# thegenemyers/DEXTRACTOR

Measured on AMD Instinct MI355X. Metric: dexqv encode input GB/s (5 QV/tag stream bytes per base; .dexqv bit-exact vs reference), higher is better.
Workload: dtype u8

## Files before the change

dextractor_amd/csrc/dx_qv.hip:

```cpp
#include "dx_internal.hpp"
#include "dx_device.hpp"

#ifndef HIST_NT
#define HIST_NT 0
#endif
#if HIST_NT
#define HIST_LOAD(p) __builtin_nontemporal_load((const u32x4_u *) (p))
#else
#define HIST_LOAD(p) (*(const u32x4_u *) (p))
#endif

#define TOK_LEN(e)  ((e) >> 26)
#define TOK_BITS(e) ((e) & 0xffffffu)
#define TOK_ESC(e)  (((e) >> 25) & 1u)
#define TOK_PACK(bits, len, esc) (((bits) & 0xffffffu) | ((uint32_t) (len) << 26) | ((esc) ? 0x2000000u : 0u))

#define QV_WIN_WORDS  512
#define QV_WIN_BITS   (32u * (QV_WIN_WORDS - 32))
#define QV_WIN_PAD    4
#ifndef QV_FLUSH_BITS
#define QV_FLUSH_BITS 8192u
#endif
#define TAG_WIN_WORDS 128
#define TAG_FLUSH_BITS 1024u

#ifndef SIZES_WAVES
#define SIZES_WAVES 4
#endif
#ifndef ENC_WAVES
#define ENC_WAVES 4
#endif
#ifndef HIST_SKIP
#define HIST_SKIP 0
#endif
#ifndef HIST_TRIM
#define HIST_TRIM 0
#endif

struct qv_args
{ const uint8_t  *text;
  const uint64_t *off;
  const uint32_t *len;
  uint64_t        n;
  uint64_t        text_bytes;
  uint32_t        pad;
  int             delChar, subChar;
  int             lossy;
  uint32_t        units;
};

static uint32_t ticket_units(uint64_t bytes, uint64_t n, uint32_t target, uint32_t least)
{ if (n == 0 || bytes == 0) return least;
  const uint64_t mean = bytes / n + 1u;
  uint64_t u = ((uint64_t) target + mean - 1u) / mean;
  return (uint32_t) (u < least ? least : (u > 4096u ? 4096u : u));
}

__device__ __forceinline__ const uint8_t *line_ptr(const qv_args &a, uint64_t r, uint32_t L, int k)
{ return a.text + a.off[r] + (uint64_t) k * ((uint64_t) L + a.pad); }

__device__ __forceinline__ bool can_overread(const qv_args &a, const uint8_t *p, uint32_t L)
{ return (uint64_t) (p - a.text) + L + 16u <= a.text_bytes; }

__device__ __forceinline__ u32x4 fetch(const uint8_t *p, uint32_t pos, uint32_t L, bool over)
{ u32x4 v = { 0u, 0u, 0u, 0u };
  if (pos < L)
    { const uint32_t left = L - pos;
      if (left >= 16u)
        v = *(const u32x4_u *) (p + pos);
      else if (over)
        { v = *(const u32x4_u *) (p + pos);
          const uint32_t m0 = left >= 4u  ? ~0u : ~(~0u << (8u * left));
          const uint32_t m1 = left >= 8u  ? ~0u : (left > 4u  ? ~(~0u << (8u * (left - 4u)))  : 0u);
          const uint32_t m2 = left >= 12u ? ~0u : (left > 8u  ? ~(~0u << (8u * (left - 8u)))  : 0u);
          const uint32_t m3 =                     (left > 12u ? ~(~0u << (8u * (left - 12u))) : 0u);
          v.x &= m0; v.y &= m1; v.z &= m2; v.w &= m3;
        }
      else
        v = load_chunk(p + pos, (int) left);
    }
  return v;
}

__device__ __forceinline__ int valid_of(uint32_t pos, uint32_t L)
{ return pos >= L ? 0 : (L - pos >= 16u ? 16 : (int) (L - pos)); }

__device__ __forceinline__ u32x4 fetch_step(const uint8_t *p, uint32_t base, uint32_t L, bool over)
{ const uint32_t pos = base + 16u * (uint32_t) lane_id();
  if (base + DX_STEP <= L)
    return *(const u32x4_u *) (p + pos);
  return fetch(p, pos, L, over);
}

#define BYTE_OF(c, b) ((chunk_word(c, (b) >> 2) >> (8 * ((b) & 3))) & 0xffu)

struct run_lds
{ uint8_t  *chunk;
  uint16_t *list;
};

__device__ __forceinline__ uint32_t run_collect(const run_lds &R, const u32x4 &c, int valid, uint32_t rc)
{ const int lane = lane_id();
  uint32_t       nr   = ~chunk_eq_mask(c, rc) & ((1u << valid) - 1u);
  const uint32_t cnt  = __popc(nr);
  const uint32_t incl = wave_incl_scan(cnt);
  uint32_t       idx  = incl - cnt;
  *(u32x4 *) (R.chunk + 16 * lane) = c;
  const uint32_t p16 = 16u * (uint32_t) lane;
  if (HIST_SKIP & 4) nr = 0;
  while (nr)
    { R.list[idx++] = (uint16_t) (p16 + (uint32_t) __builtin_ctz(nr));
      nr &= nr - 1u;
    }
  wave_sync();
  return wave_total(incl);
}

__device__ __forceinline__ uint32_t run_after(const run_lds &R, uint32_t total, uint32_t sv, uint32_t C)
{ return total ? sv - 1u - (uint32_t) R.list[total - 1] : C + sv; }


__global__ __launch_bounds__(DX_BLOCK)
void k_qv_prescan_del(qv_args a, uint64_t entry0, unsigned long long *key)
{ const int      lane  = lane_id();
  const uint64_t wave0 = (uint64_t) blockIdx.x * DX_WAVES_PER_BLK + (threadIdx.x >> 6);
  const uint64_t nwave = (uint64_t) gridDim.x * DX_WAVES_PER_BLK;

  for (uint64_t r = wave0; r < a.n; r += nwave)
    { const unsigned long long cur = __hip_atomic_load(key, __ATOMIC_RELAXED, __HIP_MEMORY_SCOPE_AGENT);
      if (entry0 + r >= (cur >> 8))
        break;
      const uint32_t L   = a.len[r];
      const uint8_t *del = line_ptr(a, r, L, 0);
      const uint8_t *tag = line_ptr(a, r, L, 1);
      bool found = false, done = false;
      for (uint32_t base = 0; base < L && !done; base += DX_STEP)
        { const uint32_t pos   = base + 16u * lane;
          const int      valid = valid_of(pos, L);
          const u32x4    c     = load_chunk(tag + pos, valid);
          const uint32_t m     = (chunk_eq_mask(c, 'n') | chunk_eq_mask(c, 'N')) & ((1u << valid) - 1u);
          const uint64_t any   = __ballot(m != 0);
          if (any)
            { const int      f = __ffsll((unsigned long long) any) - 1;
              const uint32_t k = pos + (uint32_t) (m ? __ffs(m) - 1 : 0);
              const uint32_t d = __shfl((uint32_t) (lane == f ? del[k] : 0u), f);
              done  = true;
              found = d < 128u;
              if (found && lane == f)
                atomicMin(key, ((unsigned long long) (entry0 + r) << 8) | d);
            }
        }
      if (found)
        break;
    }
}

__global__ __launch_bounds__(DX_BLOCK)
void k_qv_prescan_sub(qv_args a, long long *out )
{ __shared__ uint32_t s_hist[256];
  __shared__ uint64_t s_part[DX_BLOCK];
  __shared__ long long s_first;
  const int tid = threadIdx.x;

  s_hist[tid] = 0;
  if (tid == 0) s_first = -1;
  __syncthreads();

  uint64_t running = 0;
  for (uint64_t c0 = 0; c0 < a.n; c0 += DX_BLOCK)
    { const uint64_t i = c0 + tid;
      s_part[tid] = i < a.n ? a.len[i] : 0;
      __syncthreads();
      if (tid == 0)
        for (int k = 0; k < DX_BLOCK && c0 + k < a.n; k++)
          { running += s_part[k];
            if (running >= 100000ull)
              { s_first = (long long) (c0 + k);
                break;
              }
          }
      __syncthreads();
      if (s_first >= 0)
        break;
    }
  const long long first = s_first;
  if (first < 0)
    { if (tid == 0) { out[0] = -1; out[1] = -1; }
      return;
    }

  const int lane = lane_id(), wid = tid >> 6;
  for (long long r = wid; r <= first; r += DX_WAVES_PER_BLK)
    { const uint32_t L    = a.len[r];
      const uint8_t *sub  = line_ptr(a, (uint64_t) r, L, 4);
      const bool     over = can_overread(a, sub, L);
      for (uint32_t base = 0; base < L; base += DX_STEP)
        { const uint32_t pos   = base + 16u * (uint32_t) lane;
          const u32x4    c     = fetch(sub, pos, L, over);
          const int      valid = valid_of(pos, L);
          for (int b = 0; b < valid; b++)
            atomicAdd(&s_hist[chunk_byte(c, b)], 1u);
        }
    }
  __syncthreads();
  if (tid == 0)
    { int best = 0;
      for (int k = 1; k < 256; k++)
        if (s_hist[k] > s_hist[best])
          best = k;
      out[0] = first;
      out[1] = best;
    }
}

#ifndef TICKET_BATCH
#define TICKET_BATCH 2u
#endif
#ifndef HIST_BLOCK
#define HIST_BLOCK   1024
#endif
#ifndef HIST_PER_CU
#define HIST_PER_CU  1
#endif
#define HIST_NWAVE   (HIST_BLOCK / 64)
#ifndef HC_PLAIN
#define HC_PLAIN     32
#endif
#ifndef HC_RSYM
#define HC_RSYM      8
#endif
#ifndef HC_RUN
#define HC_RUN       8
#endif
#define HSYM_FAST    128
#define HRUN_FAST    128
#ifndef HIST_BARE_FETCH
#define HIST_BARE_FETCH 1
#endif

struct hist_lds
{ uint32_t plain[2][HSYM_FAST][HC_PLAIN];
  uint32_t rsym[2][HSYM_FAST][HC_RSYM];
  uint32_t run[2][HRUN_FAST][HC_RUN];
  uint32_t slow[6][256];
};
#define HIST_W_PLAIN (2 * HSYM_FAST * HC_PLAIN)
#define HIST_W_RSYM  (2 * HSYM_FAST * HC_RSYM)
#define HIST_W_RUN   (2 * HRUN_FAST * HC_RUN)
#define HIST_FAST_WORDS (HIST_W_PLAIN + HIST_W_RSYM + HIST_W_RUN)

template <int COLS>
__device__ __forceinline__ void hist_plain_step(const u32x4 &c, int valid, bool full, uint32_t (*h)[COLS], uint32_t *slow)
{ const uint32_t col = (uint32_t) lane_id() & (COLS - 1);
  const bool wide = __any((int) ((c.x | c.y | c.z | c.w) & 0x80808080u));
  if (full && !wide)
    {
      #pragma unroll
      for (int b = 0; b < 16; b++)
        atomicAdd(&h[BYTE_OF(c, b)][col], 1u);
    }
  else
    for (int b = 0; b < valid; b++)
      { const uint32_t x = chunk_byte(c, b);
        if (x < HSYM_FAST) atomicAdd(&h[x][col], 1u);
        else               atomicAdd(&slow[x], 1u);
      }
}

#define TOK_RUN_MAX  127u
#define TOK_BAD      0x80000000u
#define TOK_INFO     8u
#define TOK_XMARGIN  40u

struct tok_sink
{ uint16_t       *del, *sub;
  const uint64_t *off;
  uint32_t       *info;
  unsigned long long *unusable;
  uint32_t       *list;
};

__host__ __device__ __forceinline__ uint32_t tok_room(uint32_t L, uint32_t fr8)
{ return (((uint32_t) (((uint64_t) L * fr8) >> 8) + 64u + TOK_XMARGIN) + 7u) & ~7u; }

__device__ __forceinline__ uint32_t tok_exception_at(const uint32_t *slot_end, uint32_t nx, uint32_t idx)
{ uint32_t lo = 0, hi = nx;
  while (lo < hi)
    { const uint32_t mid = (lo + hi) >> 1;
      if (*(slot_end - 2 * (int) mid - 2) < idx) lo = mid + 1; else hi = mid;
    }
  return lo;
}
__device__ __forceinline__ uint32_t tok_exception(const uint32_t *slot_end, uint32_t nx, uint32_t idx)
{ return *(slot_end - 2 * (int) tok_exception_at(slot_end, nx, idx) - 1); }

__device__ __forceinline__ bool tok_unusable(const uint32_t *info, uint64_t r, int delChar, int subChar)
{ return (delChar >= 0 && (info[TOK_INFO * r] & TOK_BAD)) || (subChar >= 0 && (info[TOK_INFO * r + 1] & TOK_BAD)); }

__device__ __forceinline__ uint32_t chunk_ne_mask(const u32x4 &v, uint32_t c4 )
{ uint32_t p[4];
  #pragma unroll
  for (int i = 0; i < 4; i++)
    { const uint32_t w = chunk_word(v, i) ^ c4;
      p[i] = ((((w & 0x7f7f7f7fu) + 0x7f7f7f7fu) | w) & 0x80808080u) * 0x00204081u;
    }
  const uint32_t even = __builtin_amdgcn_perm(p[2], p[0], 0x0c0c0703u);
  const uint32_t odd  = __builtin_amdgcn_perm(p[3], p[1], 0x0c0c0703u);
  return (even >> 4) | odd;
}

__device__ __forceinline__ uint32_t chunk_byte_sel(const u32x4 &v, uint32_t selA, uint32_t selB)
{ return __builtin_amdgcn_perm(__builtin_amdgcn_perm(v.w, v.z, selA), __builtin_amdgcn_perm(v.y, v.x, selA), selB); }

__device__ __forceinline__ uint32_t wave_shr1(uint32_t v)
{ return (uint32_t) __builtin_amdgcn_update_dpp(0u, v, 0x138, 0xf, 0xf, true); }

struct tok_pend { uint64_t v; uint32_t n, at; };

__device__ __forceinline__ void tok_flush(tok_pend &p, uint16_t *tok)
{ if (4u * (uint32_t) lane_id() < p.n)
    *(u64_u *) (tok + p.at + 4u * (uint32_t) lane_id()) = p.v;
  p.n = 0;
}

__device__ __forceinline__ uint32_t tag_code(uint32_t letter)
{ const uint32_t i = min((letter & 0xdfu) - 0x41u, 31u);
  return (uint32_t) (((1ull << 4) | (2ull << 12) | (3ull << 38)) >> (2u * i)) & 3u;
}

struct hist_wave_lds
{ uint8_t  chunk[DX_STEP], tags[DX_STEP];
  uint16_t list[DX_STEP];
};
#ifndef PPC_INS
#define PPC_INS 8
#endif
#ifndef PPC_MRG
#define PPC_MRG 4
#endif
#ifndef HIST_LIST
#define HIST_LIST 512
#endif
struct hist_wave_own
{ uint32_t pi[128][PPC_INS], pm[128][PPC_MRG];
#ifndef PSC
#define PSC 1
#endif
  uint32_t ps[2][128][PSC];
#ifndef PRC
#define PRC 1
#endif
  uint32_t pr[2][128][PRC];
  uint16_t list[HIST_LIST];
};
#define EH_WORDS 384u

template <bool TAGS, bool OWN, bool LDSX>
__device__ __forceinline__ void hist_runs_step(hist_wave_lds *W, uint16_t *wlist, const u32x4 &c, const u32x4 &t, uint32_t vmask, uint32_t sv, uint32_t rc4,
                                               uint32_t &C, uint32_t &nrun, uint32_t *hs, uint32_t *slow_s,
                                               uint32_t *hr, uint32_t *slow_r, uint32_t inc,
                                               uint16_t *tok, uint32_t &ntok, uint32_t room, uint32_t &bad, uint32_t &nexc,
                                               tok_pend &pend_out)
{ constexpr uint32_t HCS = OWN ? (uint32_t) PSC : HC_RSYM, HCR = OWN ? (uint32_t) PRC : HC_RUN;
  const uint32_t lane  = (uint32_t) lane_id();
  const uint32_t nr0   = chunk_ne_mask(c, rc4) & vmask;
  const uint32_t cnt   = __popc(nr0);
  const uint32_t incl  = wave_incl_scan(cnt);
  const uint32_t total = wave_total(incl);
  nrun += sv - total;
  if (LDSX)
    { *(u32x4 *) (W->chunk + 16u * lane) = c;
      if (TAGS) *(u32x4 *) (W->tags + 16u * lane) = t;
    }
  const bool fits = OWN ? total <= (uint32_t) HIST_LIST : true;
  const bool emit = !(HIST_SKIP & 8) && !bad && fits && ntok + total + 4u * nexc <= room;
  if (!emit) bad = 1;
  const uint32_t tend  = cnt ? 16u * lane + 32u - (uint32_t) __clz(nr0) + C : 0u;
  const uint32_t imax  = wave_incl_max(tend);
  const uint32_t gmax  = __builtin_amdgcn_readlane(imax, 63);
  const uint32_t s0    = wave_shr1(imax) - (16u * lane + C);
  const uint32_t li0   = incl - cnt;
  uint32_t nr = (HIST_SKIP & 1) ? 0u : nr0, s = s0, acc = 0;
  uint16_t      *lp = wlist + (fits ? li0 : 0u);
  const uint8_t *cp = LDSX ? W->chunk + 16u * lane : (const uint8_t *) NULL;
  const uint32_t pinc = OWN ? 1u : inc;
  while (nr)
    { const uint32_t b   = (uint32_t) __builtin_ctz(nr);
      nr &= nr - 1u;
      uint32_t x, tg = 0;
      if (!LDSX)
        { const uint32_t selA = (b & 7u) | 0x0c0c0c00u, selB = ((b >> 1) & 4u) | 0x0c0c0c00u;
          x = chunk_byte_sel(c, selA, selB);
          if (TAGS) tg = chunk_byte_sel(t, selA, selB);
        }
      else
        { x = cp[b];
          if (TAGS) tg = cp[b + DX_STEP];
        }
      const uint32_t run = b - s;
      const uint32_t r7  = run < TOK_RUN_MAX ? run : TOK_RUN_MAX;
      s   = b + 1u;
      acc = max(acc, max(run, x));
#if HIST_TRIM
      const uint32_t x4 = x << 2;
      atomicAdd((uint32_t *) ((uint8_t *) hs + (x4 & (4u * (HSYM_FAST - 1))) * HCS), 1u);
      atomicAdd(&hr[r7 * HCR], pinc);
      uint32_t tk = (r7 << 9) | x4;
      if (TAGS) tk |= tag_code(tg);
#else
      atomicAdd(&hs[(x & (HSYM_FAST - 1)) * HCS], 1u);
      atomicAdd(&hr[r7 * HCR], pinc);
      uint32_t tk = x | (r7 << 7);
      if (TAGS) tk = (tk << 2) | tag_code(tg);
      else      tk <<= 2;
#endif
      *lp++ = (uint16_t) tk;
    }
  uint32_t odd = 0;
  if (__any((int) (acc >= TOK_RUN_MAX)))
    { uint32_t m = nr0, ne = 0;
      s = s0;
      while (m)
        { const uint32_t b   = (uint32_t) __builtin_ctz(m);
          m &= m - 1u;
          const uint32_t x   = LDSX ? (uint32_t) cp[b] : chunk_byte(c, (int) b);
          const uint32_t run = b - s;
          s = b + 1u;
          if (run >= TOK_RUN_MAX)
            { atomicSub(&hr[TOK_RUN_MAX * HCR], pinc);
              atomicAdd(&slow_r[run > 255u ? 255u : run], inc);
              ne++;
            }
          if (x >= HSYM_FAST)
            { atomicSub(&hs[(x & (HSYM_FAST - 1)) * HCS], 1u);
              atomicAdd(&slow_s[x], 1u);
              odd = 1;
            }
        }
      if (emit && __any((int) ne))
        { const uint32_t ince = wave_incl_scan(ne);
          uint32_t  j    = nexc + ince - ne, i = ntok + li0;
          uint32_t *xend = (uint32_t *) (tok + room + TOK_XMARGIN);
          m = nr0; s = s0;
          while (m)
            { const uint32_t b   = (uint32_t) __builtin_ctz(m);
              m &= m - 1u;
              const uint32_t run = b - s;
              s = b + 1u;
              if (run >= TOK_RUN_MAX)
                { *(xend - 2 * (int) j - 2) = i;
                  *(xend - 2 * (int) j - 1) = run;
                  j++;
                }
              i++;
            }
          nexc += wave_total(ince);
        }
      else if (OWN && __any((int) ne))
        bad = 1;
    }
  if (emit)
    { __builtin_amdgcn_wave_barrier();
      if (HIST_SKIP & 32) { }
      else if (total <= 256u)
        { pend_out.v = *(const uint64_t *) (wlist + 4u * lane); pend_out.n = total; pend_out.at = ntok; }
      else
        for (uint32_t i = 4u * lane; i < total; i += 256u)
          *(u64_u *) (tok + ntok + i) = *(const uint64_t *) (wlist + i);
      ntok += total;
      if (__any((int) odd)) bad = 1;
    }
  C = sv + C - gmax;
  __builtin_amdgcn_wave_barrier();
}

__device__ __forceinline__ void hist_plain_pair(const u32x4 &c2, const u32x4 &c3, int valid, bool full, hist_lds &H)
{ const uint32_t col = (uint32_t) lane_id() & (HC_PLAIN - 1);
  if (full && !__any((int) ((c2.x | c2.y | c2.z | c2.w | c3.x | c3.y | c3.z | c3.w) & 0x80808080u)))
    {
      #pragma unroll
      for (int b = 0; b < 16; b++)
        atomicAdd(&H.plain[0][BYTE_OF(c2, b)][col], 1u);
      #pragma unroll
      for (int b = 0; b < 16; b++)
        atomicAdd(&H.plain[1][BYTE_OF(c3, b)][col], 1u);
    }
  else
    { hist_plain_step<HC_PLAIN>(c2, valid, full, H.plain[0], H.slow[DX_INS]);
      hist_plain_step<HC_PLAIN>(c3, valid, full, H.plain[1], H.slow[DX_MRG]);
    }
}

__device__ __forceinline__ uint32_t hist_plain_pair_own(const u32x4 &c2, const u32x4 &c3, int valid, bool full, uint32_t *pi, uint32_t *pm,
                                                        uint32_t *slow_ins, uint32_t *slow_mrg)
{ uint32_t *const q0 = pi + ((uint32_t) lane_id() & (PPC_INS - 1u)), *const q1 = pm + ((uint32_t) lane_id() & (PPC_MRG - 1u));
#define OWN_ADD(q, x) atomicAdd(&(q)[((q) == q0 ? (uint32_t) PPC_INS : (uint32_t) PPC_MRG) * (x)], 1u)
  if (!__any((int) ((c2.x | c2.y | c2.z | c2.w | c3.x | c3.y | c3.z | c3.w) & 0x80808080u)))
    { if (full || valid > 0)
        {
          #pragma unroll
          for (int b = 0; b < 16; b++)
            OWN_ADD(q0, BYTE_OF(c2, b));
          #pragma unroll
          for (int b = 0; b < 16; b++)
            OWN_ADD(q1, BYTE_OF(c3, b));
          if (!full && valid < 16)
            { atomicSub(&q0[0], (uint32_t) (16 - valid));
              atomicSub(&q1[0], (uint32_t) (16 - valid));
            }
        }
      return 0;
    }
  for (int b = 0; b < valid; b++)
    { const uint32_t x = chunk_byte(c2, b), y = chunk_byte(c3, b);
      if (x < 128u) OWN_ADD(q0, x);
      else          atomicAdd(&slow_ins[x], 1u);
      if (y < 128u) OWN_ADD(q1, y);
      else          atomicAdd(&slow_mrg[y], 1u);
    }
#undef OWN_ADD
  return 1;
}

__device__ __forceinline__ uint32_t hist_bin_of(uint32_t k)
{ if (k < HIST_W_PLAIN)
    return (DX_INS + k / (HSYM_FAST * HC_PLAIN)) * 256u + (k / HC_PLAIN) % HSYM_FAST;
  k -= HIST_W_PLAIN;
  if (k < HIST_W_RSYM)
    return (k / (HSYM_FAST * HC_RSYM) ? DX_SUB : DX_DEL) * 256u + (k / HC_RSYM) % HSYM_FAST;
  k -= HIST_W_RSYM;
  if (k < HIST_W_RUN)
    return (4u + k / (HRUN_FAST * HC_RUN)) * 256u + (k / HC_RUN) % HRUN_FAST;
  return k - HIST_W_RUN;
}

__device__ __forceinline__ uint32_t hist_copies_of(uint32_t k)
{ return k < HIST_W_PLAIN ? HC_PLAIN : (k < HIST_W_PLAIN + HIST_W_RSYM ? HC_RSYM : HC_RUN); }

struct meta_row { const uint8_t *base; uint32_t stride, pad; };

__device__ __forceinline__ uint32_t meta_load(const meta_row *s_meta, uint32_t words, uint64_t r)
{ uint32_t v = 0;
  const uint32_t lane = (uint32_t) lane_id();
  if (lane < words)
    { const meta_row m = s_meta[lane];
      v = *(const uint32_t *) (m.base + r * m.stride);
    }
  return v;
}
#define META(m, k)   ((uint32_t) __builtin_amdgcn_readlane((int) (m), (int) (k)))
#define META64(m, k) ((uint64_t) META(m, k) | ((uint64_t) META(m, (k) + 1) << 32))

struct scan_dev
{ int32_t   delChar, subChar;
  long long del_first, sub_first;
  uint32_t  inst;
  uint32_t  share8;
};
#define SCAN_G     0u
#define SCAN_A     1u
#define SCAN_B     2u
#define SCAN_NOTOK 3u
#define SCAN_MISS  0x100u

template <bool FAST, bool OWNTOK> struct hist_smem;
template <> struct hist_smem<false, false> { hist_lds H; hist_wave_lds W[HIST_NWAVE]; };
template <> struct hist_smem<true, true>   { uint32_t slow[6][256]; hist_wave_own W[HIST_NWAVE]; };
struct hist_wave_plain { uint32_t pi[128][PPC_INS], pm[128][PPC_MRG]; uint16_t list[DX_STEP]; };
template <> struct hist_smem<true, false>
{ uint32_t slow[6][256];
  uint32_t rsym[2][HSYM_FAST][HC_RSYM], run[2][HRUN_FAST][HC_RUN];
  hist_wave_plain W[HIST_NWAVE];
};

template <bool FAST, bool OWNTOK>
__global__ __launch_bounds__(HIST_BLOCK, (HIST_NWAVE * HIST_PER_CU + 3) / 4)
void k_qv_hist(qv_args a, uint64_t entry0, long long del_first, long long sub_first,
               unsigned long long *g_hist , unsigned long long *g_tot, uint32_t *ticket, tok_sink ts, uint32_t *eh ,
               const scan_dev *sd , uint64_t tok_cap ,
               const uint32_t *orig )
{ __shared__ __attribute__((aligned(16))) hist_smem<FAST, OWNTOK> S;
  if (sd != NULL)
    { if (sd->inst != (FAST ? (OWNTOK ? SCAN_A : SCAN_B) : SCAN_G) || ts.off[a.n] > tok_cap)
        return;
      a.delChar = sd->delChar; a.subChar = sd->subChar;
      del_first = sd->del_first; sub_first = sd->sub_first;
    }
  typedef hist_smem<false, false> smem_g;
  typedef hist_smem<true, true>   smem_a;
  typedef hist_smem<true, false>  smem_b;
  const int      lane  = lane_id();
  const int      tid   = threadIdx.x;
  const int      wid   = tid >> 6;
  uint32_t (*const slow)[256] = !FAST ? ((smem_g *) (void *) &S)->H.slow : (OWNTOK ? ((smem_a *) (void *) &S)->slow : ((smem_b *) (void *) &S)->slow);
  hist_lds      *const Hp = FAST ? (hist_lds *) NULL : &((smem_g *) (void *) &S)->H;
  hist_wave_lds *const Wl = FAST ? (hist_wave_lds *) NULL : &((smem_g *) (void *) &S)->W[wid];
  hist_wave_own *const Wo = FAST && OWNTOK ? &((smem_a *) (void *) &S)->W[wid] : (hist_wave_own *) NULL;
  smem_b        *const Sb = FAST && !OWNTOK ? (smem_b *) (void *) &S : (smem_b *) NULL;
  uint32_t *const piw = !FAST ? (uint32_t *) NULL : (OWNTOK ? &Wo->pi[0][0] : &Sb->W[wid].pi[0][0]);
  uint32_t *const pmw = !FAST ? (uint32_t *) NULL : (OWNTOK ? &Wo->pm[0][0] : &Sb->W[wid].pm[0][0]);
  uint16_t      *const wlist = !FAST ? Wl->list : (OWNTOK ? Wo->list : Sb->W[wid].list);
  uint32_t *const words = (uint32_t *) (void *) &S;
  const uint32_t  nwords = sizeof(S) / 4;
  const bool      toks  = FAST || ts.del != NULL;
  constexpr bool OT = FAST && OWNTOK;
  uint32_t (*const rsymp)[HSYM_FAST][HC_RSYM] = FAST ? (OWNTOK ? (uint32_t (*)[HSYM_FAST][HC_RSYM]) NULL : Sb->rsym) : Hp->rsym;
  uint32_t (*const runp)[HRUN_FAST][HC_RUN]   = FAST ? (OWNTOK ? (uint32_t (*)[HRUN_FAST][HC_RUN]) NULL : Sb->run) : Hp->run;
  uint32_t *const hs0 = OT ? &Wo->ps[0][0][(uint32_t) lane & (PSC - 1)] : &rsymp[0][0][(uint32_t) lane & (HC_RSYM - 1)];
  uint32_t *const hs4 = OT ? &Wo->ps[1][0][(uint32_t) lane & (PSC - 1)] : &rsymp[1][0][(uint32_t) lane & (HC_RSYM - 1)];
  uint32_t *const hr0 = OT ? &Wo->pr[0][0][(uint32_t) lane & (PRC - 1)] : &runp[0][0][(uint32_t) lane & (HC_RUN - 1)];
  uint32_t *const hr4 = OT ? &Wo->pr[1][0][(uint32_t) lane & (PRC - 1)] : &runp[1][0][(uint32_t) lane & (HC_RUN - 1)];
  const uint32_t  rc0 = (uint32_t) (a.delChar & 0xff) * 0x01010101u, rc4 = (uint32_t) (a.subChar & 0xff) * 0x01010101u;

#define HM_WORDS 8u
  __shared__ __attribute__((aligned(16))) meta_row s_meta[HM_WORDS];
  if (tid < (int) HM_WORDS)
    { meta_row m;
      if      (tid == 0) { m.base = (const uint8_t *) a.len;                   m.stride = 4u; }
      else if (tid < 3)  { m.base = (const uint8_t *) a.off + 4 * (tid - 1);   m.stride = 8u; }
      else if (tid < 7)  { m.base = (const uint8_t *) ts.off + 4 * (tid - 3);  m.stride = 8u; }
      else               { m.base = (const uint8_t *) orig;                    m.stride = 4u; }
      if ((tid >= 3 && tid < 7 && !(FAST || ts.del != NULL)) || (tid == 7 && orig == NULL))
        { m.base = (const uint8_t *) a.len; m.stride = 0u; }
      m.pad = 0;
      s_meta[tid] = m;
    }
  for (uint32_t k = tid; k < nwords; k += HIST_BLOCK) words[k] = 0;
  __syncthreads();

  uint64_t tot = 0, since = 0;
  uint32_t mpre = 0;
  uint64_t mfor = ~0ull;
  for (uint64_t r0 = next_unit(ticket, a.units), nxt; r0 < a.n; r0 = nxt)
  { nxt = next_unit(ticket, a.units);
    for (uint64_t r = r0; r < r0 + a.units && r < a.n; r++)
    { const uint32_t mw = mfor == r ? mpre : meta_load(s_meta, HM_WORDS, r);
      { const uint64_t rn = r + 1 < r0 + a.units && r + 1 < a.n ? r + 1 : nxt;
        mfor = rn;
        if (rn < a.n) mpre = meta_load(s_meta, HM_WORDS, rn);
      }
      const uint32_t  L = META(mw, 0);
      const long long g = (long long) (entry0 + (orig ? (uint64_t) META(mw, 7) : r));
      const bool drun = FAST || (a.delChar >= 0 && (toks || g >= del_first));
      const bool srun = FAST || (a.subChar >= 0 && (toks || g >= sub_first));
      const uint32_t dinc = (a.delChar >= 0 && g >= del_first) ? 1u : 0u, sinc = (a.subChar >= 0 && g >= sub_first) ? 1u : 0u;
      const uint8_t *p0 = a.text + META64(mw, 1);
      const uint64_t pitch = (uint64_t) L + a.pad;
      const uint8_t *p1 = p0 + pitch, *p2 = p1 + pitch, *p3 = p2 + pitch, *p4 = p3 + pitch;
      const bool over = can_overread(a, p4, L);
      uint32_t C0 = 0, C4 = 0, n0 = 0, n4 = 0;
      uint16_t *tk0 = NULL, *tk4 = NULL;
      uint32_t  nt0 = 0, nt4 = 0, room = 0, bad0 = 0, bad4 = 0, nx0 = 0, nx4 = 0;
      tok_pend  pd0 = { 0ull, 0u, 0u }, pd4 = { 0ull, 0u, 0u };
      if (toks)
        { const uint64_t t0 = META64(mw, 3);
          room = (uint32_t) (META64(mw, 5) - t0) - TOK_XMARGIN;
          if (drun) tk0 = ts.del + t0;
          if (srun) tk4 = ts.sub + t0;
        }
      const bool tags = FAST || tk0 != NULL;

      uint32_t pos = 16u * lane;
      u32x4 c0 = fetch(p0, pos, L, over), c4 = fetch(p4, pos, L, over);
      u32x4 t1 = c0;
      if (tags) t1 = fetch(p1, pos, L, over);
      for (uint32_t base = 0; base < L; base += DX_STEP)
        { const uint32_t np = pos + DX_STEP;
          __builtin_amdgcn_s_waitcnt(0x0F70);
          if (toks)
            { tok_flush(pd0, tk0);
              tok_flush(pd4, tk4);
            }
          u32x4 c2, c3, d0, d4, u1 = c0;
          if (HIST_BARE_FETCH && base + DX_STEP <= L)
            { c2 = HIST_LOAD(p2 + pos); c3 = HIST_LOAD(p3 + pos); }
          else
            { c2 = fetch(p2, pos, L, over); c3 = fetch(p3, pos, L, over); }
          if (HIST_BARE_FETCH && base + 2u * DX_STEP <= L)
            { d0 = HIST_LOAD(p0 + np); d4 = HIST_LOAD(p4 + np);
              if (tags) u1 = HIST_LOAD(p1 + np);
            }
          else
            { d0 = fetch(p0, np, L, over); d4 = fetch(p4, np, L, over);
              if (tags) u1 = fetch(p1, np, L, over);
            }
          const uint32_t sv    = L - base >= DX_STEP ? DX_STEP : L - base;
          const bool     full  = sv == DX_STEP;
          const int      valid = valid_of(pos, L);
          const uint32_t vmask = (1u << valid) - 1u;
          if (HIST_SKIP & 16) { }
          else if (drun) hist_runs_step<true, OT, !FAST>(Wl, wlist, c0, t1, vmask, sv, rc0, C0, n0, hs0, slow[DX_DEL], hr0, slow[DX_DRUN],
                                                    dinc, tk0, nt0, tk0 != NULL ? room : 0u, bad0, nx0, pd0);
          else      hist_plain_step<HC_RSYM>(c0, valid, full, Hp->rsym[0], slow[DX_DEL]);
          if (HIST_SKIP & 16) { }
          else if (srun) hist_runs_step<false, OT, !FAST>(Wl, wlist, c4, c4, vmask, sv, rc4, C4, n4, hs4, slow[DX_SUB], hr4, slow[DX_SRUN],
                                                     sinc, tk4, nt4, tk4 != NULL ? room : 0u, bad4, nx4, pd4);
          else      hist_plain_step<HC_RSYM>(c4, valid, full, Hp->rsym[1], slow[DX_SUB]);
          if (HIST_SKIP & 2) { }
          else if (FAST) bad0 |= hist_plain_pair_own(c2, c3, valid, full, piw, pmw, slow[DX_INS], slow[DX_MRG]);
          else           hist_plain_pair(c2, c3, valid, full, *Hp);
          c0 = d0; c4 = d4; t1 = u1;
          pos = np;
        }
      tok_flush(pd0, tk0);
      tok_flush(pd4, tk4);
      if (FAST)
        {
          __builtin_amdgcn_wave_barrier();
          uint32_t *e32 = eh + (uint64_t) r * EH_WORDS;
          const u32x4 zero = { 0u, 0u, 0u, 0u };
          #pragma unroll
          for (int k = 0; k < 2; k++)
            { const int cp = k == 0 ? PPC_INS : PPC_MRG;
              u32x4 *w = (u32x4 *) ((k == 0 ? piw : pmw) + 2 * lane * cp);
              uint32_t ce = 0, co = 0;
              if (cp == 2)
                { const u32x4 v = w[0];
                  w[0] = zero;
                  ce = v.x + v.y; co = v.z + v.w;
                }
              else
                {
                  #pragma unroll
                  for (int j = 0; j < cp / 4; j++)
                    { const u32x4 v0 = w[j], v1 = w[cp / 4 + j];
                      w[j] = zero; w[cp / 4 + j] = zero;
                      ce += v0.x + v0.y + v0.z + v0.w; co += v1.x + v1.y + v1.z + v1.w;
                    }
                }
              e32[64 * k + lane] = (ce & 0xffffu) | (co << 16);
              if (ce | co)
                { atomicAdd(&slow[DX_INS + k][2 * lane], ce);
                  atomicAdd(&slow[DX_INS + k][2 * lane + 1], co);
                }
            }
          #pragma unroll
          for (int k = 0; k < (OT ? 4 : 0); k++)
            { uint32_t v0, v1;
              if (k < 2)
                { uint32_t *w = &Wo->ps[k][2 * lane][0];
                  v0 = 0; v1 = 0;
                  #pragma unroll
                  for (int j = 0; j < PSC; j++)
                    { v0 += w[j]; v1 += w[PSC + j];
                      w[j] = 0; w[PSC + j] = 0;
                    }
                }
              else
                { uint32_t *w = &Wo->pr[k - 2][2 * lane][0];
                  v0 = 0; v1 = 0;
                  #pragma unroll
                  for (int j = 0; j < PRC; j++)
                    { v0 += w[j]; v1 += w[PRC + j];
                      w[j] = 0; w[PRC + j] = 0;
                    }
                }
              e32[128 + 64 * k + lane] = (v0 & 0xffffu) | (v1 << 16);
              const int      tab = k == 0 ? DX_DEL : (k == 1 ? DX_SUB : (k == 2 ? DX_DRUN : DX_SRUN));
              const uint32_t on  = k == 2 ? dinc : (k == 3 ? sinc : 1u);
              if (on && (v0 | v1))
                { atomicAdd(&slow[tab][2 * lane], v0);
                  atomicAdd(&slow[tab][2 * lane + 1], v1);
                }
            }
          __builtin_amdgcn_wave_barrier();
        }
      if (drun)
        { if (dinc && C0 > 0 && lane == 0) atomicAdd(&slow[DX_DRUN][C0 > 255u ? 255u : C0], 1u);
          if (lane == 0 && n0) atomicAdd(&slow[DX_DEL][a.delChar], n0);
        }
      if (srun)
        { if (sinc && C4 > 0 && lane == 0) atomicAdd(&slow[DX_SRUN][C4 > 255u ? 255u : C4], 1u);
          if (lane == 0 && n4) atomicAdd(&slow[DX_SUB][a.subChar], n4);
        }
      if (toks)
        { if (FAST && (bad0 || bad4)) { bad0 = 1; bad4 = 1; }
          if (lane == 0)
            { uint32_t *w = ts.info + TOK_INFO * r;
              w[0] = nt0 | ((bad0 || !drun) ? TOK_BAD : 0u);
              w[1] = nt4 | ((bad4 || !srun) ? TOK_BAD : 0u);
              w[2] = C0;
              w[3] = C4;
              w[4] = nx0;
              w[5] = nx4;
              w[6] = (FAST && L > 65535u ? 1u : 0u) |
                     (FAST && !OWNTOK ? 2u : 0u);
            }
          if (((drun && bad0) || (srun && bad4)) && lane == 0)
            ts.list[atomicAdd(ts.unusable, 1ull)] = (uint32_t) r;
        }
      tot   += L;
      since += L;
      if (since >= (1ull << 26))
        { if (FAST)
            { for (uint32_t k = lane; k < 6u * 256u; k += 64)
                { const uint32_t v = atomicExch(&slow[0][k], 0u);
                  if (v) atomicAdd(&g_hist[k], (unsigned long long) v);
                }
              if (!OWNTOK)
                { for (uint32_t k = lane; k < 2u * HSYM_FAST * HC_RSYM; k += 64)
                    { const uint32_t v = atomicExch(&(&Sb->rsym[0][0][0])[k], 0u);
                      if (v) atomicAdd(&g_hist[(k / (HSYM_FAST * HC_RSYM) ? DX_SUB : DX_DEL) * 256u + (k / HC_RSYM) % HSYM_FAST], (unsigned long long) v);
                    }
                  for (uint32_t k = lane; k < 2u * HRUN_FAST * HC_RUN; k += 64)
                    { const uint32_t v = atomicExch(&(&Sb->run[0][0][0])[k], 0u);
                      if (v) atomicAdd(&g_hist[(4u + k / (HRUN_FAST * HC_RUN)) * 256u + (k / HC_RUN) % HRUN_FAST], (unsigned long long) v);
                    }
                }
            }
          else
            for (uint32_t k = lane; k < sizeof(hist_lds) / 4; k += 64)
              { const uint32_t v = atomicExch(&words[k], 0u);
                if (v) atomicAdd(&g_hist[hist_bin_of(k)], (unsigned long long) v);
              }
          since = 0;
        }
    }
  }
  if (lane == 0 && tot)
    atomicAdd(g_tot, (unsigned long long) tot);
  __syncthreads();
  if (FAST && !OWNTOK)
    { for (uint32_t k = tid; k < 2u * HSYM_FAST; k += HIST_BLOCK)
        { uint32_t v = 0;
          for (uint32_t j = 0; j < HC_RSYM; j++) v += (&Sb->rsym[0][0][0])[k * HC_RSYM + j];
          if (v) atomicAdd(&g_hist[(k / HSYM_FAST ? DX_SUB : DX_DEL) * 256u + k % HSYM_FAST], (unsigned long long) v);
        }
      for (uint32_t k = tid; k < 2u * HRUN_FAST; k += HIST_BLOCK)
        { uint32_t v = 0;
          for (uint32_t j = 0; j < HC_RUN; j++) v += (&Sb->run[0][0][0])[k * HC_RUN + j];
          if (v) atomicAdd(&g_hist[(4u + k / HRUN_FAST) * 256u + k % HRUN_FAST], (unsigned long long) v);
        }
    }
  if (!FAST)
    for (uint32_t w8 = tid; w8 < HIST_FAST_WORDS / 8u; w8 += HIST_BLOCK)
      { uint32_t v = 0;
        for (uint32_t j = 0; j < 8u; j++)
          v += words[w8 * 8u + ((j + (uint32_t) lane) & 7u)];
        if (v) atomicAdd(&g_hist[hist_bin_of(w8 * 8u)], (unsigned long long) v);
      }
  for (uint32_t k = tid; k < 6 * 256; k += HIST_BLOCK)
    { const uint32_t v = slow[0][k];
      if (v) atomicAdd(&g_hist[k], (unsigned long long) v);
    }
}

__global__ void k_scan_state(const unsigned long long *key, const long long *sub, dx_qv_params in, int want_del, int want_sub, scan_dev *sd)
{ if (threadIdx.x != 0 || blockIdx.x != 0) return;
  scan_dev d;
  d.delChar = in.delChar; d.subChar = in.subChar; d.del_first = in.del_first; d.sub_first = in.sub_first;
  if (want_del && *key != ~0ull)
    { d.delChar   = (int32_t) (*key & 0xff);
      d.del_first = (long long) (*key >> 8);
    }
  if (want_sub && sub[0] >= 0)
    { d.subChar   = (int32_t) sub[1];
      d.sub_first = sub[0];
    }
  d.inst = 0; d.share8 = 0;
  *sd = d;
}

__global__ __launch_bounds__(DX_BLOCK)
void k_qv_density(qv_args a, uint64_t stride, unsigned long long *cnt, const scan_dev *sd )
{ if (sd != NULL) { a.delChar = sd->delChar; a.subChar = sd->subChar; }
  const int      lane = lane_id();
  const uint64_t w    = (uint64_t) blockIdx.x * DX_WAVES_PER_BLK + (threadIdx.x >> 6);
  const uint64_t r    = w * stride;
  if (r >= a.n) return;
  const uint32_t L = a.len[r], S = L < 4096u ? L : 4096u;
  #pragma unroll 1
  for (int k = 0; k < 2; k++)
    { const int rc = k == 0 ? a.delChar : a.subChar;
      if (rc < 0) continue;
      const uint8_t *p = line_ptr(a, r, L, k == 0 ? 0 : 4);
      uint32_t tokens = 0;
      for (uint32_t j = (uint32_t) lane; j < S; j += 64u)
        tokens += p[j] != (uint8_t) rc ? 1u : 0u;
      tokens = wave_sum(tokens);
      if (lane == 0)
        { atomicAdd(&cnt[2 * k], (unsigned long long) S);
          atomicAdd(&cnt[2 * k + 1], (unsigned long long) tokens);
        }
    }
}

__device__ __forceinline__ uint32_t tok_share_of(const unsigned long long *cnt)
{ const double fd = cnt[0] ? (double) cnt[1] / (double) cnt[0] : 0.0, fs = cnt[2] ? (double) cnt[3] / (double) cnt[2] : 0.0;
  const double f  = 1.5 * (fd > fs ? fd : fs) + 0.05;
  const uint32_t fr8 = (uint32_t) (256.0 * f + 0.999);
  return fr8 < 64u ? 64u : (fr8 > 256u ? 256u : fr8);
}

#define HIST_SHARE_A 110u
__global__ __launch_bounds__(DX_BLOCK)
void k_tok_rooms(const uint32_t *len, uint64_t n, unsigned long long *cnt, uint32_t *room, scan_dev *sd, uint32_t guess, int shared_tokens)
{ const uint64_t i = (uint64_t) blockIdx.x * DX_BLOCK + threadIdx.x;
  const uint32_t fr8 = tok_share_of(cnt);
  if (i == 0)
    { cnt[4] = fr8;
      if (sd != NULL)
        { const uint32_t inst = sd->delChar < 0 && sd->subChar < 0 ? SCAN_NOTOK
                              : (sd->delChar >= 0 && sd->subChar >= 0 ? (fr8 <= HIST_SHARE_A && !shared_tokens ? SCAN_A : SCAN_B) : SCAN_G);
          sd->share8 = fr8;
          sd->inst   = inst | (inst != guess ? SCAN_MISS : 0u);
        }
    }
  if (i < n) room[i] = tok_room(len[i], fr8);
}

__device__ __forceinline__ void load_tables(uint32_t (*s_tok)[256], const uint32_t *g_tok)
{ for (int k = threadIdx.x; k < DX_TOK_WORDS; k += (int) blockDim.x)
    (&s_tok[0][0])[k] = g_tok[k];
  __syncthreads();
}

__device__ __forceinline__ uint32_t pad_extra(uint64_t T, uint32_t last)
{ const uint32_t olen = (uint32_t) T & 31u;
  const uint32_t llen = (uint32_t) (T - last) & 31u;
  if (olen > 0)
    return (llen > 16u && olen > llen) ? 1u : 0u;
  return (T > 0 && llen > 16u) ? 1u : 0u;
}

__device__ __forceinline__ uint32_t last_piece_plain(const uint32_t *tab, const uint8_t *p, uint32_t L, uint32_t mask)
{ if (L == 0) return 0;
  const uint32_t e = tab[p[L - 1] & mask];
  return TOK_ESC(e) ? 8u : TOK_LEN(e);
}

__device__ __forceinline__ uint32_t last_piece_byte(const uint32_t *tab, uint32_t last_byte, uint32_t L, uint32_t mask)
{ if (L == 0) return 0;
  const uint32_t e = tab[last_byte & mask];
  return TOK_ESC(e) ? 8u : TOK_LEN(e);
}

__device__ __forceinline__ uint32_t seg_bytes(uint64_t T, uint32_t last)
{ return 4u * ((uint32_t) (T >> 5) + (((uint32_t) T & 31u) ? 1u : 0u) + pad_extra(T, last)); }

__device__ __forceinline__ uint32_t run_token_len(const uint32_t *rtab, uint32_t run)
{ const uint32_t e = rtab[run > 255u ? 255u : run];
  return TOK_LEN(e) + (TOK_ESC(e) ? 16u : 0u);
}

struct size_tabs
{ uint8_t  len[6][256];
  uint16_t inner[2][256];
};

__device__ __forceinline__ void load_size_tables(size_tabs &t, const uint32_t *g_tok, int delChar, int subChar)
{ for (int k = threadIdx.x; k < 6 * 256; k += (int) blockDim.x)
    { const uint32_t e = g_tok[k];
      uint32_t l = TOK_LEN(e) + ((k >= 4 * 256 && TOK_ESC(e)) ? 16u : 0u);
      if ((delChar >= 0 && k == DX_DEL * 256 + delChar) || (subChar >= 0 && k == DX_SUB * 256 + subChar))
        l = 0;
      (&t.len[0][0])[k] = (uint8_t) l;
    }
  __syncthreads();
  for (int k = threadIdx.x; k < 2 * 256; k += (int) blockDim.x)
    { const uint8_t *rl = t.len[4 + (k >> 8)];
      uint32_t m = (uint32_t) k & 0xffu, sum = 0;
      int prev = -1;
      for (int b = 0; b < 8; b++)
        if ((m >> b) & 1u)
          { if (prev >= 0) sum += rl[b - prev - 1];
            prev = b;
          }
      (&t.inner[0][0])[k] = (uint16_t) sum;
    }
  __syncthreads();
}

__device__ __forceinline__ uint32_t bits_syms_step(const u32x4 &c, int valid, const uint8_t *len, uint32_t m4)
{ uint32_t acc = 0;
  #pragma unroll
  for (int b = 0; b < 16; b++)
    acc += len[((chunk_word(c, b >> 2) & m4) >> (8 * (b & 3))) & 0xffu];
  return acc - (16u - (uint32_t) valid) * len[0];
}

__device__ __forceinline__ uint32_t bits_runs_step(const u32x4 &c, int valid, uint32_t sv, uint32_t rc, uint32_t &C,
                                                   uint32_t &nonrun, const uint8_t *rlen, const uint16_t *inner)
{ const uint32_t nr = ~chunk_eq_mask(c, rc) & ((1u << valid) - 1u);
  const uint32_t lo = nr & 0xffu, hi = nr >> 8;
  const uint32_t p0 = 16u * (uint32_t) lane_id();
  const uint32_t incl = wave_incl_max(nr ? p0 + 32u - (uint32_t) __clz(nr) : 0u);
  const uint32_t prev = __builtin_amdgcn_update_dpp(0u, incl, 0x138, 0xf, 0xf, true);
  uint32_t acc = (uint32_t) inner[lo] + (uint32_t) inner[hi];
  if (lo && hi)
    acc += rlen[(uint32_t) __clz(lo) - 24u + (uint32_t) __ffs(hi) - 1u];
  if (nr)
    { const uint32_t run = p0 + (uint32_t) __ffs(nr) - 1u - (prev ? prev : 0u - C);
      acc += rlen[run > 255u ? 255u : run];
    }
  nonrun += __popc(nr);
  const uint32_t end = __builtin_amdgcn_readlane(incl, 63);
  C = end ? sv - end : C + sv;
  return acc;
}

__global__ __launch_bounds__(DX_BLOCK, SIZES_WAVES)
void k_qv_sizes(qv_args a, const uint32_t *g_tok, const uint64_t *hdr_off, uint32_t *seg ,
                uint32_t *rec_size, uint32_t *ticket,
                const uint32_t *only_list, const unsigned long long *only_count, uint64_t first_entry, const uint32_t *only_info)
{ __shared__ uint32_t  s_tok[6][256];
  __shared__ size_tabs s_t;
  load_tables(s_tok, g_tok);
  load_size_tables(s_t, g_tok, a.delChar, a.subChar);
// ... 1617 lines not shown
```

Measured before the change: 2179.

## Carry token tail in registers so global token stores cover whole 64-token lines

After: 2179, median of 2. No clear change (-0.0%).

```diff
diff --git a/dextractor_amd/csrc/dx_qv.hip b/dextractor_amd/csrc/dx_qv.hip
--- a/dextractor_amd/csrc/dx_qv.hip
+++ b/dextractor_amd/csrc/dx_qv.hip
@@ -280,8 +280,9 @@
   uint32_t       *list;
 };
 
+#define TOK_LINE     64u
 __host__ __device__ __forceinline__ uint32_t tok_room(uint32_t L, uint32_t fr8)
-{ return (((uint32_t) (((uint64_t) L * fr8) >> 8) + 64u + TOK_XMARGIN) + 7u) & ~7u; }
+{ return (((uint32_t) (((uint64_t) L * fr8) >> 8) + 64u + TOK_XMARGIN) + TOK_LINE - 1u) & ~(TOK_LINE - 1u); }
 
 __device__ __forceinline__ uint32_t tok_exception_at(const uint32_t *slot_end, uint32_t nx, uint32_t idx)
 { uint32_t lo = 0, hi = nx;
@@ -315,7 +316,7 @@
 __device__ __forceinline__ uint32_t wave_shr1(uint32_t v)
 { return (uint32_t) __builtin_amdgcn_update_dpp(0u, v, 0x138, 0xf, 0xf, true); }
 
-struct tok_pend { uint64_t v; uint32_t n, at; };
+struct tok_pend { uint64_t v, t; uint32_t n, at; };
 
 __device__ __forceinline__ void tok_flush(tok_pend &p, uint16_t *tok)
 { if (4u * (uint32_t) lane_id() < p.n)
@@ -323,6 +324,11 @@
   p.n = 0;
 }
 
+__device__ __forceinline__ void tok_flush_tail(const tok_pend &p, uint16_t *tok, uint32_t ntok)
+{ if (!(HIST_SKIP & 32) && 4u * (uint32_t) lane_id() < (ntok & (TOK_LINE - 1u)))
+    *(u64_u *) (tok + (ntok & ~(TOK_LINE - 1u)) + 4u * (uint32_t) lane_id()) = p.t;
+}
+
 __device__ __forceinline__ uint32_t tag_code(uint32_t letter)
 { const uint32_t i = min((letter & 0xdfu) - 0x41u, 31u);
   return (uint32_t) (((1ull << 4) | (2ull << 12) | (3ull << 38)) >> (2u * i)) & 3u;
@@ -330,7 +336,7 @@
 
 struct hist_wave_lds
 { uint8_t  chunk[DX_STEP], tags[DX_STEP];
-  uint16_t list[DX_STEP];
+  uint16_t list[DX_STEP + TOK_LINE];
 };
 #ifndef PPC_INS
 #define PPC_INS 8
@@ -351,7 +357,7 @@
 #define PRC 1
 #endif
   uint32_t pr[2][128][PRC];
-  uint16_t list[HIST_LIST];
+  uint16_t list[HIST_LIST + TOK_LINE];
 };
 #define EH_WORDS 384u
 
@@ -381,7 +387,10 @@
   const uint32_t s0    = wave_shr1(imax) - (16u * lane + C);
   const uint32_t li0   = incl - cnt;
   uint32_t nr = (HIST_SKIP & 1) ? 0u : nr0, s = s0, acc = 0;
-  uint16_t      *lp = wlist + (fits ? li0 : 0u);
+  const uint32_t held = ntok & (TOK_LINE - 1u);
+  if (4u * lane < held) *(uint64_t *) (wlist + 4u * lane) = pend_out.t;
+  __builtin_amdgcn_wave_barrier();
+  uint16_t      *lp = wlist + (fits ? held + li0 : 0u);
   const uint8_t *cp = LDSX ? W->chunk + 16u * lane : (const uint8_t *) NULL;
   const uint32_t pinc = OWN ? 1u : inc;
   while (nr)
@@ -461,12 +470,16 @@
     }
   if (emit)
     { __builtin_amdgcn_wave_barrier();
+      const uint32_t whole = (held + total) & ~(TOK_LINE - 1u);
       if (HIST_SKIP & 32) { }
-      else if (total <= 256u)
-        { pend_out.v = *(const uint64_t *) (wlist + 4u * lane); pend_out.n = total; pend_out.at = ntok; }
       else
-        for (uint32_t i = 4u * lane; i < total; i += 256u)
-          *(u64_u *) (tok + ntok + i) = *(const uint64_t *) (wlist + i);
+        { if (whole <= 256u)
+            { pend_out.v = *(const uint64_t *) (wlist + 4u * lane); pend_out.n = whole; pend_out.at = ntok - held; }
+          else
+            for (uint32_t i = 4u * lane; i < whole; i += 256u)
+              *(u64_u *) (tok + (ntok - held) + i) = *(const uint64_t *) (wlist + i);
+          pend_out.t = *(const uint64_t *) (wlist + whole + 4u * (lane & 15u));
+        }
       ntok += total;
       if (__any((int) odd)) bad = 1;
     }
@@ -566,7 +579,7 @@
 template <bool FAST, bool OWNTOK> struct hist_smem;
 template <> struct hist_smem<false, false> { hist_lds H; hist_wave_lds W[HIST_NWAVE]; };
 template <> struct hist_smem<true, true>   { uint32_t slow[6][256]; hist_wave_own W[HIST_NWAVE]; };
-struct hist_wave_plain { uint32_t pi[128][PPC_INS], pm[128][PPC_MRG]; uint16_t list[DX_STEP]; };
+struct hist_wave_plain { uint32_t pi[128][PPC_INS], pm[128][PPC_MRG]; uint16_t list[DX_STEP + TOK_LINE]; };
 template <> struct hist_smem<true, false>
 { uint32_t slow[6][256];
   uint32_t rsym[2][HSYM_FAST][HC_RSYM], run[2][HRUN_FAST][HC_RUN];
@@ -651,7 +664,7 @@
       uint32_t C0 = 0, C4 = 0, n0 = 0, n4 = 0;
       uint16_t *tk0 = NULL, *tk4 = NULL;
       uint32_t  nt0 = 0, nt4 = 0, room = 0, bad0 = 0, bad4 = 0, nx0 = 0, nx4 = 0;
-      tok_pend  pd0 = { 0ull, 0u, 0u }, pd4 = { 0ull, 0u, 0u };
+      tok_pend  pd0 = { 0ull, 0ull, 0u, 0u }, pd4 = { 0ull, 0ull, 0u, 0u };
       if (toks)
         { const uint64_t t0 = META64(mw, 3);
           room = (uint32_t) (META64(mw, 5) - t0) - TOK_XMARGIN;
@@ -704,6 +717,10 @@
         }
       tok_flush(pd0, tk0);
       tok_flush(pd4, tk4);
+      if (toks)
+        { tok_flush_tail(pd0, tk0, nt0);
+          tok_flush_tail(pd4, tk4, nt4);
+        }
       if (FAST)
         {
           __builtin_amdgcn_wave_barrier();
```
